# SingleZombie/AFLDM

Measured on AMD Instinct MI355X. Metric: denoise-steps/sec + ms/step, FFHQ-256 AF-UNet, batch 64 @1/2/4/8 GPU, higher is better.
Workload: dtype bf16; 1 GPU; FFHQ-256 AF-UNet single denoise step, batch 64 per GPU (BASELINE configs[1]); batch_per_gpu=64, global_batch=64, hip_graph=True, latents_finite=True

## Files before the change

afldm_amd/csrc/conv.hip:

```cpp
#include <stdlib.h>

#include "conv_common.hpp"

namespace afldm {

__device__ __forceinline__ int swz(int row) { return (4 - ((row >> 2) & 3)) & 3; }

template <typename T>
__device__ __forceinline__ void epilogue_store(const ConvP& p, int m, int n, f32x4 v) {
  const T* temb = (const T*)p.temb;
  const T* res = (const T*)p.residual;
  T* y = (T*)p.y;
  const int HW = p.H * p.W;
  const int b = m / HW;
  if (p.y2 && n >= p.split_n) {
    T* y2 = (T*)p.y2;
    const int pix = m - b * HW, c2 = p.Cout - p.split_n;
    for (int r = 0; r < 4 && n + r < p.Cout; ++r) {
      float sv = v[r] + (p.bias ? p.bias[n + r] : 0.f);
      y2[((size_t)b * c2 + (n + r - p.split_n)) * HW + pix] = from_f32<T>(sv);
    }
    return;
  }
  if (n + 3 < p.Cout && p.vec_ok) {
// ... 1845 lines not shown
    const int eo = 16 / (int)sizeof(T);
    const int hw = a->H * a->W;
    const bool cm = a->out_mode == 1 || a->y2;
    p.stage_ok = ((a->out_mode == 1 || a->y_ld % eo == 0) && (!a->residual || a->res_ld % eo == 0) &&
                  (!a->temb || a->temb_stride % eo == 0) && (!cm || hw % eo == 0) && (!a->y2 || a->split_n % eo == 0) &&
                  !(cm && a->residual)) ? 1 : 0;
    static const int s_nostage = getenv("AFLDM_CONV_NOSTAGE") ? atoi(getenv("AFLDM_CONV_NOSTAGE")) : 0;
    if (s_nostage) p.stage_ok = 0;
  }
  {
    static const int s_mfast = getenv("AFLDM_CONV_MFAST") ? atoi(getenv("AFLDM_CONV_MFAST")) : -1;
    p.m_fast = s_mfast >= 0 ? s_mfast : ((long long)a->Cout * a->KS * a->KS > (long long)p.M ? 1 : 0);
  }
  p.xcd_gn = 0;
  p.y_norm = nullptr; p.ngamma = nullptr; p.nbeta = nullptr; p.ncpg = 1; p.neps = 0.f;
  p.x_c8 = a->x_layout == 1 ? 1 : 0;
  p.y_c8 = a->y_layout == 1 ? 1 : 0;
  p.w_nt = 0;
  p.sc_x1 = a->sc_x1; p.sc_x2 = a->sc_x2; p.sc_w = a->sc_w;
  p.sc_C1 = a->sc_x1 ? a->sc_C1 : 0; p.sc_C2 = a->sc_x1 ? a->sc_C2 : 0;
}

template <typename T>
static bool shortcut_ok(const afldm_conv_args* a) {
  const int kstep = KCH_DEFAULT * epr<T>();
  const long long M = (long long)a->B * a->H * a->W, Csc = (long long)a->sc_C1 + a->sc_C2;
  if (!a->sc_x1 || !a->sc_w || a->sc_C1 <= 0 || a->sc_C2 < 0 || a->sc_C1 % kstep || a->sc_C2 % kstep || (a->sc_C2 > 0) != (a->sc_x2 != nullptr))
    return false;
  if (!aligned16(a->sc_x1) || !aligned16(a->sc_x2) || !aligned16(a->sc_w)) return false;
  if (a->KS != 3 || a->residual || a->defer_reduce || a->w_batch_stride || a->y_norm || a->y2 || a->out_mode != 0) return false;
  const long long cmax = a->sc_C1 > a->sc_C2 ? a->sc_C1 : a->sc_C2;
  if (M >= (1ll << 28) || M * cmax * (long long)sizeof(T) >= (1ll << 31) || (long long)a->Cout * Csc * (long long)sizeof(T) >= (1ll << 31)) return false;
  if (lin_wreg_bm(a) || skinny_stats_splits(a)) return false;
  const Exec ex = resolve_exec<T>(a);
  return ex.pl.kind == 0 && kVariants[ex.vid].ver == 6 && ex.splitk == 1 && !ex.fused && conv3h_shortcut_ok(ex.vid);
}

template <typename T>
static bool c8_ok(const afldm_conv_args* a) {
  if (sizeof(T) != 2 || a->C2 != 0 || a->x2 || a->y2 || a->out_mode != 0 || a->y_norm || a->y_ld != a->Cout || a->Cout % 8 || a->C1 % 64) return false;
  if (a->w_batch_stride || a->defer_reduce || a->KS != 3 || lin_wreg_bm(a) || skinny_stats_splits(a)) return false;
  const Exec ex = resolve_exec<T>(a);
  if (ex.pl.kind != 0 || kVariants[ex.vid].ver != 6 || ex.splitk != 1 || ex.fused) return false;
  if (a->stats_out) {
    int S = 0;
    if (stats_mode<T>(a, ex, &S) != ST_EPILOGUE) return false;
  }
  return a->H == a->W && a->W <= 32 && a->H * a->W >= kVariants[ex.vid].bm;
}

template <typename T>
static int conv_dispatch(const afldm_conv_args* a, hipStream_t st) {
  AFLDM_REQUIRE((a->x_layout == 0 && a->y_layout == 0) || c8_ok<T>(a), AFLDM_ESHAPE,
                "afldm_conv2d: x_layout / y_layout = 1 (8-channel blocks) is not available for this problem (afldm_conv2d_c8_ok)");
  AFLDM_REQUIRE(!a->sc_x1 || shortcut_ok<T>(a), AFLDM_ESHAPE,
                "afldm_conv2d: the folded shortcut (sc_x1 / sc_w) is not available for this problem (afldm_conv2d_shortcut_ok)");
  ConvP p;
  fill_convp<T>(a, p);
// ... 186 lines not shown
  const afldm_conv_args* a = &ac;
  const Exec e = a->dtype == AFLDM_F32 ? resolve_exec<float>(a) : resolve_exec<bf16>(a);
  if (skinny_stats_splits(a)) return -16;
  if (e.pl.kind != 0) return -1 - e.pl.kind;
  return e.vid | (e.splitk << 8) | (e.fused << 16);
}

extern "C" int afldm_conv2d_c8_ok(const afldm_conv_args* a) {
  if (!a || a->dtype != AFLDM_BF16 || conv_validate(a) || conv_batch_chunk(a) != a->B) return 0;
  return c8_ok<bf16>(a) ? 1 : 0;
}

extern "C" int afldm_conv2d_norm_ok(const afldm_conv_args* a) {
  if (!a || a->dtype != AFLDM_BF16 || conv_batch_chunk(a) != a->B || !a->stats_out) return 0;
  if (lin_wreg_bm(a) || skinny_stats_splits(a)) return 0;
  const Exec e = resolve_exec<bf16>(a);
  int S = 0;
  const int smode = stats_mode<bf16>(a, e, &S);
  return norm_fusable<bf16>(a, e, smode) ? 1 : 0;
}

extern "C" int afldm_conv2d_shortcut_ok(const afldm_conv_args* a) {
  if (!a || conv_validate(a) || conv_batch_chunk(a) != a->B) return 0;
  if (a->dtype == AFLDM_BF16) return shortcut_ok<bf16>(a) ? 1 : 0;
  if (a->dtype == AFLDM_F32) return shortcut_ok<float>(a) ? 1 : 0;
  return 0;
}

extern "C" int afldm_conv2d_stats_splits(const afldm_conv_args* a0) {
  if (!a0 || (a0->dtype != AFLDM_F32 && a0->dtype != AFLDM_BF16)) return 0;
  const afldm_conv_args ac = conv_chunk_args(a0, conv_batch_chunk(a0));
  const afldm_conv_args* a = &ac;
  int S = 0;
  if (a->dtype == AFLDM_F32) stats_mode<float>(a, resolve_exec<float>(a), &S);
  else stats_mode<bf16>(a, resolve_exec<bf16>(a), &S);
  return S;
}

extern "C" size_t afldm_conv2d_workspace(const afldm_conv_args* a0) {
  if (!a0 || (a0->dtype != AFLDM_F32 && a0->dtype != AFLDM_BF16)) return 0;
  const afldm_conv_args ac = conv_chunk_args(a0, conv_batch_chunk(a0));
  const afldm_conv_args* a = &ac;
  if (lin_wreg_bm(a) || skinny_stats_splits(a)) return 0;
  Plan pl = make_plan(a, a->dtype == AFLDM_F32 ? 16 : 32);
  if (pl.kind != 0 || pl.splitk <= 1) return 0;
  return (size_t)pl.splitk * a->B * a->H * a->W * a->Cout * sizeof(float);
}

// ... 30 lines not shown
```

afldm_amd/csrc/conv3h.hip:

```cpp
#include "conv3h_tile.hpp"

namespace afldm {

template <typename T, int BM, int W_, int BN, int WGM, int WGN, int NPROD, int STAGES, int MINW, int MF, int TPS, bool SUB = false>
__global__ void __launch_bounds__((WGM * WGN + NPROD) * 64, MINW) k_conv3h(ConvP p) {
  extern __shared__ __attribute__((aligned(16))) char smem[];
#define H3_BX blockIdx.x
#define H3_NBX gridDim.x
#define H3_BZ blockIdx.z
#define H3_PATCH_AUX 0
#define H3_PRODUCER_EXIT return;
#include "conv3h_body.inc"
#undef H3_PRODUCER_EXIT
#undef H3_BX
#undef H3_NBX
#undef H3_BZ
#undef H3_PATCH_AUX
}

template <int BM, int W_, int BN, int WGM, int WGN, bool SUB>
__global__ void __launch_bounds__((WGM * WGN + 4) * 64, (WGM * WGN + 4 + 3) / 4) k_conv3h_pers(ConvP p) {
  typedef bf16 T;
  typedef Mma<T> MM;
  typedef typename MM::Chunk Chunk;
// ... 374 lines not shown
  const int k = variant - kConv3hFirst;
  if (k < 0 || k >= kNumH3) return false;
  const H3Variant& v = kH3[k];
  if (v.bm == 0) return false;
  const int kstep = 128 / dtype_size;
  const int eo = 16 / dtype_size;
  const int HW = p.H * p.W;
  const int z = p.splitk > 0 ? p.splitk : 1;
  const bool tile_ok = HW % v.bm == 0 || (v.bm % HW == 0 && (z > 1 || dtype_size == 2));
  const bool plane_ok = v.sub ? (p.W > v.w && p.W % v.w == 0 && p.H % (v.bm / v.w) == 0 && z == 1) : (p.W == v.w && p.H == p.W && tile_ok);
  if ((k == 22 || k == 23) && !(dtype_size == 2 && z == 1 && HW % v.bm == 0 && p.C1 / kstep >= 2 && (!p.temb || p.temb_mod > 0))) return false;
  if (k >= 24 && dtype_size != 2) return false;
  return p.KS == 3 && p.C2 == 0 && plane_ok && p.M % v.bm == 0 && p.Cout % v.bn == 0 &&
         p.C1 % kstep == 0 && (p.C1 / kstep) % z == 0 && p.out_mode == 0 && !p.y2 && p.y_ld % eo == 0 &&
         (!p.residual || p.res_ld % eo == 0) && (!p.temb || (p.temb_stride % eo == 0 && p.temb_mod % eo == 0)) &&
         (long long)p.M * p.C1 * dtype_size < (1ll << 31) && (long long)p.Cout * 9 * p.C1 * dtype_size < (1ll << 31) &&
         p.Cout % 4 == 0 && aligned16(p.y) && aligned16(p.x1) && aligned16(p.w);
}

bool conv3h_shortcut_ok(int variant) {
  const int k = variant - kConv3hFirst;
  if (k < 0 || k >= kNumH3 || k == 22 || k == 23) return false;
  const H3Variant& v = kH3[k];
  return v.bm != 0 && v.tps == 1 && !v.sub && !(v.bm == 256 && v.w == 16);
}

template <typename T, int BM, int W_, int BN, int WGM, int WGN, int MF, int TPS, int STAGES = 3, bool SUB = false, int NPROD = 4, int MINW_ = 0>
static void launch_h3(const ConvP& p0, hipStream_t st) {
  constexpr int NWC = WGM * WGN;
  constexpr int MINW = MINW_ > 0 ? MINW_ : (NWC + NPROD + 3) / 4;
  constexpr int ROWS = BM / W_, SEG = ROWS < W_ ? ROWS : W_, NSEG = ROWS / SEG;
  constexpr int NPI = (NSEG * (SEG + 2) * (W_ + 2) + 7) / 8;
  constexpr int lds = 2 * NPI * 1024 + STAGES * TPS * BN * 128;
  static_assert(lds <= 160 * 1024, "LDS");
  ConvP p = p0;
  p.tiles_n = p.Cout / BN;
  if (p.splitk < 1) p.splitk = 1;
  const int tiles_m = p.M / BM, tiles = tiles_m * p.tiles_n;
  {
    static const int s_gn = getenv("AFLDM_CONV3H_GN") ? atoi(getenv("AFLDM_CONV3H_GN")) : -1;
    const double xb = (double)p.M * p.C1, wb = 9.0 * p.Cout * p.C1;
    int best = 0;
    double best_cost = xb + 8.0 * wb;
    for (int gn = 2; gn <= 8; gn *= 2) {
      if (tiles % 8 || p.tiles_n % gn || tiles_m % (8 / gn)) continue;
      const double c = xb * gn + wb * (8 / gn);
      if (c < 0.9 * best_cost) best = gn, best_cost = c;
// ... 81 lines not shown
```

afldm_amd/csrc/conv3h_body.inc:

```
  typedef Mma<T> MM;
  typedef typename MM::Chunk Chunk;
  constexpr int NWC = WGM * WGN;
  constexpr int EPC = MM::EPC, KSTEP = 8 * EPC, ESZ = (int)sizeof(T);
  constexpr int WMS = BM / WGM, WNS = BN / WGN, TM = WMS / MF, TN = WNS / MF;
  constexpr int ROWS = BM / W_, SEG = ROWS < W_ ? ROWS : W_, NSEG = ROWS / SEG;
  constexpr int PW = W_ + 2, PR = NSEG * (SEG + 2), NPQ = PR * PW, NPI = (NPQ + 7) / 8;
  constexpr int PATCH = NPI * 1024;
  constexpr int SPC = 9 / TPS;
  constexpr int WIT = BN / 8;
  constexpr int WI = TPS * WIT, WPW = WI / NPROD, PPW = (NPI + NPROD - 1) / NPROD;
  constexpr int W_TAP = BN * 128, W_STAGE = TPS * W_TAP;
  constexpr int LDS_TOTAL = 2 * PATCH + STAGES * W_STAGE;
  constexpr unsigned OOB = 0x80000000u;
  static_assert(MF == 16 || MF == 32, "MFMA flavour");
  static_assert(TPS == 1 || TPS == 3, "taps per step");
  static_assert(BM % W_ == 0 && ROWS % SEG == 0 && WI % NPROD == 0 && WMS % MF == 0 && WNS % MF == 0, "tile shape");
  static_assert((STAGES - 2) * WPW + PPW < 64, "vmcnt is a 6-bit counter");

  const int tid = threadIdx.x, lane = tid & 63;
  const int wave_all = __builtin_amdgcn_readfirstlane(tid >> 6);
  const bool is_producer = wave_all >= NWC;
  const int li = lane & (MF - 1), lg = lane / MF;

  int tile_m, tile_n;
  if (p.xcd_gn > 0) {
    const int xcd = H3_BX & 7, j = H3_BX >> 3;
    const int gn = p.xcd_gn, tn_per = p.tiles_n / gn, tm_per = (H3_NBX / p.tiles_n) / (8 / gn);
    const int xm = xcd / gn, xn = xcd - xm * gn;
    const int lm = j / tn_per, ln = j - lm * tn_per;
    tile_m = xm * tm_per + lm;
    tile_n = xn * tn_per + ln;
  } else {
    const int tile = xcd_remap(H3_BX, H3_NBX);
    tile_m = tile / p.tiles_n;
    tile_n = tile - tile_m * p.tiles_n;
  }
  static_assert(!SUB || (NSEG == 1 && TPS == 1), "sub-tiled planes: one segment per tile");
  const int n0 = tile_n * BN;
  const int Ct = p.C1, HW = SUB ? p.H * p.W : W_ * W_;
  const int ncb = Ct / KSTEP;
  const int ks = H3_BZ;
  const int cb_lo = (ncb * ks) / p.splitk, cb_hi = (ncb * (ks + 1)) / p.splitk;
  constexpr bool HAS_SC = TPS == 1 && !SUB && !(BM == 256 && W_ == 16);
  const int nsc = (HAS_SC && p.sc_x1) ? (p.sc_C1 + p.sc_C2) / KSTEP : 0;
  const int cb_end = cb_hi + nsc;
  const int Gm = (cb_hi - cb_lo) * SPC, G = Gm + nsc;
  int m0, b_tile, oh0, ow0 = 0, sp_tile;
  if constexpr (SUB) {
    const int tw = p.W / W_, tps = (p.H / ROWS) * tw;
    b_tile = tile_m / tps;
    sp_tile = tile_m - b_tile * tps;
    const int ty = sp_tile / tw;
    oh0 = ty * ROWS;
    ow0 = (sp_tile - ty * tw) * W_;
    m0 = b_tile * HW + oh0 * p.W + ow0;
  } else {
    m0 = tile_m * BM;
    b_tile = m0 / HW;
    oh0 = NSEG == 1 ? (m0 - b_tile * HW) / W_ : 0;
    sp_tile = (m0 - b_tile * HW) / BM;
  }
  auto gpix = [&](int tp) -> int {
    if constexpr (SUB) return m0 + (tp / W_) * p.W + (tp % W_);
    else return m0 + tp;
  };

  if (is_producer) {
// ... 22 lines not shown
        ok = q < NPQ && pc >= 1 && pc <= W_ && ih >= 0 && ih < W_;
        pixel = m0 + (sg * SEG + jj - 1) * W_ + (pc - 1);
      }
      if (p.x_c8) {
        const int bb = pixel / HW, pp = pixel - bb * HW;
        poff[i] = ok ? (((unsigned)(bb * (Ct / EPC) + c) * (unsigned)HW + (unsigned)pp) * (unsigned)EPC) * ESZ : OOB;
      } else {
        poff[i] = ok ? ((unsigned)pixel * (unsigned)Ct + (unsigned)(c * EPC)) * ESZ : OOB;
      }
    }
#pragma unroll
    for (int i = 0; i < WPW; ++i) {
      const int j = wave + NPROD * i;
      const int tis = j / WIT, r = 8 * (j - tis * WIT) + (lane >> 3);
      const int c = h_chunk_at<MF>(lane & 7, h_sw_rows<MF>(r));
      woff[i] = (((unsigned)(n0 + r) * 9u + (unsigned)tis) * (unsigned)Ct + (unsigned)(c * EPC)) * ESZ;
    }
    const int Csc = p.sc_C1 + p.sc_C2;
    __amdgpu_buffer_rsrc_t rws = __builtin_amdgcn_make_buffer_rsrc((void*)p.sc_w, 0, (int)((long long)p.Cout * Csc * ESZ), 0x00020000);
    int is_g = 0, is_st = 0, is_cb = cb_lo, is_slot = 0;
    auto issue_weights = [&]() {
      char* sbase = smem + 2 * PATCH + is_slot * W_STAGE;
      if (HAS_SC && is_g >= Gm && is_g < G) {
        const unsigned so = (unsigned)((is_g - Gm) * KSTEP * ESZ);
#pragma unroll
        for (int i = 0; i < WPW; ++i) {
          const int r = 8 * (wave + NPROD * i) + (lane >> 3);
          const unsigned wo = ((unsigned)(n0 + r) * (unsigned)Csc + (unsigned)(h_chunk_at<MF>(lane & 7, h_sw_rows<MF>(r)) * EPC)) * ESZ;
          lds_ptr_t dst = (lds_ptr_t)(sbase + (wave + NPROD * i) * 1024);
          if (p.w_nt) __builtin_amdgcn_raw_ptr_buffer_load_lds(rws, dst, 16, (int)wo, (int)so, 0, 2);
          else __builtin_amdgcn_raw_ptr_buffer_load_lds(rws, dst, 16, (int)wo, (int)so, 0, 0);
        }
      } else {
        const unsigned so = is_g < Gm ? (unsigned)((is_st * TPS * Ct + is_cb * KSTEP) * ESZ) : OOB;
#pragma unroll
        for (int i = 0; i < WPW; ++i) {
          lds_ptr_t dst = (lds_ptr_t)(sbase + (wave + NPROD * i) * 1024);
          if (p.w_nt) __builtin_amdgcn_raw_ptr_buffer_load_lds(rw, dst, 16, (int)woff[i], (int)so, 0, 2);
          else __builtin_amdgcn_raw_ptr_buffer_load_lds(rw, dst, 16, (int)woff[i], (int)so, 0, 0);
        }
      }
      ++is_g;
      if (++is_st == SPC) {
        is_st = 0;
        ++is_cb;
      }
      is_slot = is_slot + 1 == STAGES ? 0 : is_slot + 1;
    };
    auto issue_patch = [&](int cb) {
      char* sbase = smem + ((cb - cb_lo) & 1) * PATCH;
      if (HAS_SC && cb >= cb_hi) {
        const int c0 = (cb - cb_hi) * KSTEP;
        const bool in1 = c0 < p.sc_C1;
        const int Cs = in1 ? p.sc_C1 : p.sc_C2;
        __amdgpu_buffer_rsrc_t rs = __builtin_amdgcn_make_buffer_rsrc(const_cast<void*>(in1 ? p.sc_x1 : p.sc_x2), 0,
                                                                     (int)((long long)p.M * Cs * ESZ), 0x00020000);
        const unsigned so = (unsigned)((in1 ? c0 : c0 - p.sc_C1) * ESZ);
#pragma unroll
        for (int i = 0; i < PPW; ++i) {
          const int q = 8 * pj[i] + (lane >> 3);
          const int c = h_chunk_at<MF>(lane & 7, h_sw_patch<MF, W_>(q));
          const int pr = q / PW, pc = q - pr * PW;
          const int sg = pr / (SEG + 2), jj = pr - sg * (SEG + 2);
          const bool in = q < NPQ && pc >= 1 && pc <= W_ && jj >= 1 && jj <= SEG;
          const int pixel = m0 + (sg * SEG + jj - 1) * W_ + (pc - 1);
          const unsigned off = in ? ((unsigned)pixel * (unsigned)Cs + (unsigned)(c * EPC)) * ESZ : OOB;
          lds_ptr_t dst = (lds_ptr_t)(sbase + pj[i] * 1024);
          __builtin_amdgcn_raw_ptr_buffer_load_lds(rs, dst, 16, (int)off, (int)so, 0, 0);
        }
        return;
      }
      const unsigned so = p.x_c8 ? (unsigned)cb * (unsigned)(KSTEP * ESZ) * (unsigned)HW : (unsigned)(cb * KSTEP * ESZ);
#pragma unroll
      for (int i = 0; i < PPW; ++i) {
        lds_ptr_t dst = (lds_ptr_t)(sbase + pj[i] * 1024);
        __builtin_amdgcn_raw_ptr_buffer_load_lds(rx, dst, 16, (int)poff[i], (int)so, 0, H3_PATCH_AUX);
      }
    };
    issue_patch(cb_lo);
#pragma unroll
    for (int s = 0; s < STAGES - 1; ++s) issue_weights();
    int st = 0, cb = cb_lo, since = STAGES;
    bool fresh = false;
    for (int g = 0; g < G; ++g) {
      if (fresh) wait_vmcnt<(STAGES >= 3 ? WPW : 0)>();
      else if (since <= STAGES - 1) wait_vmcnt<(STAGES - 2) * WPW + PPW>();
      else wait_vmcnt<(STAGES - 2) * WPW>();
      __builtin_amdgcn_s_barrier();
      ++since;
      fresh = false;
      if (!(p.dbg & 1)) {
        if (HAS_SC && cb >= cb_hi) {
          if (cb + 1 < cb_end) {
            issue_patch(cb + 1);
            fresh = true;
            since = STAGES;
          }
          issue_weights();
        } else {
          issue_weights();
          if (st == 0 && cb + 1 < cb_end) {
            issue_patch(cb + 1);
            since = 1;
          }
        }
      }
      if ((HAS_SC && cb >= cb_hi) || ++st == SPC) {
        st = 0;
        ++cb;
      }
// ... 102 lines not shown
          }
#pragma unroll
          for (int kk = 0; kk < NKK; ++kk) {
            Chunk a[TN], b[TM];
#pragma unroll
            for (int t = 0; t < TN; ++t) a[t] = ld16<Chunk>(sW + ti * W_TAP + ((a_off0 + t * MF * 128) ^ (kk << 5)));
#pragma unroll
            for (int t = 0; t < TM; ++t) b[t] = ld16<Chunk>(sP + (bo[t] ^ (kk << 5)));
#pragma unroll
            for (int tn = 0; tn < TN; ++tn)
#pragma unroll
              for (int tm = 0; tm < TM; ++tm) {
                if constexpr (MF == 16) MM::mma(acc[tn][tm], a[tn], b[tm]);
                else Mma32<T>::mma(acc[tn][tm], a[tn], b[tm]);
              }
            __builtin_amdgcn_sched_barrier(0);
          }
        }
      }
      step_end();
    };
    auto k_step = [&](auto ST) {
      constexpr int sst = decltype(ST)::value;
      if (!(p.dbg & 2)) {
        const char* sP = smem + pbuf * PATCH;
        const char* sW = smem + 2 * PATCH + slot * W_STAGE;
        int boff[TPS][TM];
#pragma unroll
        for (int ti = 0; ti < TPS; ++ti) {
          const int tap = st * TPS + ti;
          const int tapoff = (tap / 3) * PW + (tap - (tap / 3) * 3);
#pragma unroll
          for (int t = 0; t < TM; ++t) {
            if constexpr (sst >= 0) boff[ti][t] = btab[sst * TPS + ti][t];
            else boff[ti][t] = frag_off(qb[t] + tapoff);
          }
        }
        constexpr int NPH = TPS * NKK, NG = NPH * TN, AD = 3;
        Chunk af[NG], bf[NPH][TM];
        auto lda = [&](int i) {
          const int ph = i / TN, ti = ph / NKK, kk = ph - ti * NKK;
#ifdef AFLDM_H3_NOLOAD
          return Chunk{};
#endif
          return ld16<Chunk>(sW + ti * W_TAP + ((a_off0 + (i - ph * TN) * MF * 128) ^ (kk << 5)));
        };
        auto ldb = [&](int ph, int t) {
          const int ti = ph / NKK, kk = ph - ti * NKK;
#ifdef AFLDM_H3_NOLOAD
          return Chunk{};
#endif
          return ld16<Chunk>(sP + (boff[ti][t] ^ (kk << 5)));
        };
#pragma unroll
        for (int t = 0; t < TM; ++t) bf[0][t] = ldb(0, t);
#pragma unroll
        for (int i = 0; i < AD; ++i) af[i] = lda(i);
        __builtin_amdgcn_sched_barrier(0);
#pragma unroll
        for (int i = 0; i < NG; ++i) {
          if (i + AD < NG) af[i + AD] = lda(i + AD);
// ... 23 lines not shown
        constexpr int c = decltype(C)::value;
        __builtin_amdgcn_s_barrier();
        if (c > 0) res_add(c - 1);
        res_issue(c);
        if constexpr (TPS == 3) k_step_plain(C);
        else k_step_plain(RT{});
      };
      static_assert(TPS == 1 || NRS == SPC, "peeled steps = one channel block");
      peeled(std::integral_constant<int, 0>{});
      peeled(std::integral_constant<int, 1>{});
      peeled(std::integral_constant<int, 2>{});
      if constexpr (NRS > 3) {
        peeled(std::integral_constant<int, 3>{});
        peeled(std::integral_constant<int, 4>{});
        peeled(std::integral_constant<int, 5>{});
        peeled(std::integral_constant<int, 6>{});
        peeled(std::integral_constant<int, 7>{});
      }
      static_assert(NRS == 3 || NRS == 8, "peeled steps");
      res_add(NRS - 1);
      g = NRS;
    }
    if constexpr (TPS == 3) {
      for (; g < G; g += 3) {
        __builtin_amdgcn_s_barrier();
        k_step(std::integral_constant<int, 0>{});
        __builtin_amdgcn_s_barrier();
        k_step(std::integral_constant<int, 1>{});
        __builtin_amdgcn_s_barrier();
        k_step(std::integral_constant<int, 2>{});
      }
    } else {
      for (; g < Gm; ++g) {
        __builtin_amdgcn_s_barrier();
        k_step(RT{});
      }
      for (; HAS_SC && g < G; ++g) {
        __builtin_amdgcn_s_barrier();
        st = 4;
        k_step(RT{});
        st = 0;
        pbuf ^= 1;
      }
    }
  }

  if (p.dbg & 8) return;
  if constexpr (ESZ == 2) {
    if (p.splitk == 1) {
      constexpr int NTC = NWC * 64, EO = 8, CPR = BN / EO, RPI = NTC / CPR, OROW = BN + 8;
      constexpr int SB_BYTES = ((NSEG * BN * 4 + 1023) / 1024) * 1024, HWT = BM / NSEG;
      static_assert(SB_BYTES + BM * OROW * 2 <= LDS_TOTAL && RPI * BN * 8 <= LDS_TOTAL, "staging tile");
      float* sB = reinterpret_cast<float*>(smem);
// ... 267 lines not shown
```

afldm_amd/csrc/conv_common.hpp:

```cpp
#pragma once
#include "common.hpp"

namespace afldm {

struct ConvP {
  const void* x1;
  const void* x2;
  const void* w;
  const float* bias;
  const void* temb;
  const void* residual;
  void* y;
  void* y2;
  float* ws;
  int split_n;
  int C1, C2, B, H, W, Cout, KS;
  int temb_stride, res_ld, y_ld, out_mode;
  int temb_mod;
  int M;
  int ksteps;
  int splitk;
  int tiles_n;
  int vec_ok;
  int tap_inner;
// ... 9 lines not shown
  void* y_norm;
  const float* ngamma;
  const float* nbeta;
  int ncpg;
  float neps;
  int x_c8, y_c8;
  int w_nt;
  const void* sc_x1;
  const void* sc_x2;
  const void* sc_w;
  int sc_C1, sc_C2;
};

typedef __attribute__((address_space(3))) void* lds_ptr_t;

template <int N>
__device__ __forceinline__ void wait_vmcnt() {
  asm volatile("s_waitcnt vmcnt(%0)" ::"n"(N) : "memory");
}

constexpr int kConv3hFirst = 41;
bool conv3h_supported(int variant, int dtype_size, const ConvP& p);
bool conv3h_shortcut_ok(int variant);
int conv3h_tile(int variant, int* bm, int* bn);
void conv3h_launch(int variant, int dtype_size, const ConvP& p, hipStream_t st);
bool conv3h_plan(const afldm_conv_args* a, ConvP* p, int* variant);

}
```

afldm_amd/models/blocks.py:

```python
import math

import os

import torch
import torch.nn as nn

from .. import aql, ops

_SC_ORDER = int(os.environ.get("AFLDM_SHORTCUT_ORDER", "0"))
_C8_EDGES = int(os.environ.get("AFLDM_C8_EDGES", "5"))
_SC_FOLD = os.environ.get("AFLDM_NO_SHORTCUT_FOLD", "0") != "1"


def _pair(x):
    return x if isinstance(x, tuple) else (x, None)


class PackedMixin:

    def _packed(self, key, build):
        cache = self.__dict__.setdefault("_afldm_cache", {})
        if key not in cache:
            cache[key] = build()
        return cache[key]

    def _invalidate(self):
        self.__dict__.pop("_afldm_cache", None)


def invalidate_packed(module: nn.Module):
    for m in module.modules():
        m.__dict__.pop("_afldm_cache", None)


# ... 338 lines not shown
        cin = x1.shape[-1] + (0 if x2 is None else x2.shape[-1])
        key = (B, N, cin, x1.device, int(temb_stride))
        cache = self.__dict__.setdefault("_afldm_c8", {})
        if key not in cache:
            w1, b1 = packed_conv(self.conv1, x1.dtype)
            w2, b2 = packed_conv(self.conv2, x1.dtype)
            a_in = torch.empty((B, N, N, cin), dtype=x1.dtype, device=x1.device)
            h_in = torch.empty((B, N, N, self.out_channels), dtype=x1.dtype, device=x1.device)
            cache[key] = (ops.conv2d_c8_ok(a_in, w1, b1, temb=temb_proj, temb_stride=temb_stride),
                          ops.conv2d_c8_ok(h_in, w2, b2, residual=h_in))
        return cache[key]

    def _sc_bias(self):
        cache = self.__dict__.setdefault("_afldm_cache", {})
        if "sc_bias" not in cache:
            b = torch.zeros(self.out_channels, dtype=torch.float64, device=self.conv2.weight.device)
            for conv in (self.conv2, self.conv_shortcut):
                if conv.bias is not None:
                    b += conv.bias.detach().double()
            cache["sc_bias"] = b.float().contiguous()
        return cache["sc_bias"]

    def _sc_fold_plan(self, input_tensor, c8):
        if (not _SC_FOLD or self.conv_shortcut is None or tuple(self.conv_shortcut.kernel_size) != (1, 1)
                or tuple(self.conv2.kernel_size) != (3, 3)):
            return False
        x1, x2 = _pair(input_tensor)
        if x1.ndim != 4 or x1.shape[1] != x1.shape[2]:
            return False
        B, N = x1.shape[0], x1.shape[1]
        key = (B, N, x1.shape[-1], None if x2 is None else x2.shape[-1], x1.dtype, x1.device, bool(c8))
        cache = self.__dict__.setdefault("_afldm_sc_fold", {})
        if key not in cache:
            w2, _ = packed_conv(self.conv2, x1.dtype)
            wsc, _ = packed_conv(self.conv_shortcut, x1.dtype)
            h_in = torch.empty((B, N, N, self.out_channels), dtype=x1.dtype, device=x1.device)
            if c8:
                h_in.c8 = True
            cache[key] = ops.conv2d_shortcut_ok(h_in, w2, self._sc_bias(), (x1, x2, wsc))
        return cache[key]

    def _conv2_sc_folded(self, h, input_tensor, next_gn):
        x1, x2 = _pair(input_tensor)
        w2, _ = packed_conv(self.conv2, h.dtype)
        wsc, _ = packed_conv(self.conv_shortcut, h.dtype)
        kw = {}
        if next_gn is not None:
            gamma, beta = packed_norm(next_gn)
            kw["norm_out"] = (gamma, beta, next_gn.num_groups, next_gn.eps)
        out = ops.conv2d(h, w2, self._sc_bias(), want_stats=True, shortcut=(x1, x2, wsc), **kw)
        hn = getattr(out, "norm_applied", None)
        if hn is not None:
            out.gn_applied = (hn, next_gn)
        return out

    def _norm_act(self, norm, x, out_c8=False, out_const=False):
        from ..af_modules.af_blocks import WarpedNonlinearity
        x1, x2 = _pair(x)
        gamma, beta = packed_norm(norm)
        stats = ops.gn_stats(x1, norm.num_groups, x2=x2)
        if isinstance(self.nonlinearity, WarpedNonlinearity):
            if self.nonlinearity.fused_silu:
                return ops.af_act(x1, x2, stats, gamma, beta, norm.num_groups, norm.eps, out_c8=out_c8, out_const=out_const)
            return self.nonlinearity(ops.gn_apply(x1, stats, gamma, beta, norm.num_groups, norm.eps, act=0, x2=x2))
        return ops.gn_apply(x1, stats, gamma, beta, norm.num_groups, norm.eps, act=1, x2=x2)

    def _norm_act_conv(self, norm, x, conv, force=False, **kw):
        from ..af_modules.af_blocks import WarpedNonlinearity
        x1, x2 = _pair(x)
        if (isinstance(self.nonlinearity, WarpedNonlinearity) and self.nonlinearity.fused_silu and x1.ndim == 4
# ... 13 lines not shown
            return None
        B, N, _, Cin = h.shape
        conv, norm = self.conv1, self.norm2
        Cout = conv.out_channels
        if tuple(conv.kernel_size) != (3, 3) or Cout % norm.num_groups or Cin % 8 or Cout % 8:
            return None
        if N == 2 and not os.environ.get("AFLDM_NO_DENSE2X2"):
            w2, _ = packed_conv_dense2x2(conv, h.dtype, Cin, 0)
            got = ops.conv2d_slabs(h.reshape(B, 4 * Cin), w2)
        else:
            w, _ = packed_conv(conv, h.dtype)
            got = ops.conv2d_slabs(h, w)
        if got is None:
            return None
        slabs, nslab = got
        gamma, beta = packed_norm(norm)
        cache = conv.__dict__.setdefault("_afldm_cache", {})
        if "bias_f32" not in cache:
            cache["bias_f32"] = None if conv.bias is None else conv.bias.detach().to(torch.float32).contiguous()
        bias = cache["bias_f32"]
        return ops.af_act_slabs(slabs, nslab, bias, temb_proj, temb_stride, gamma, beta, norm.num_groups, norm.eps,
                                B, N, Cout, h.dtype)

    def _conv2_to_next_norm_fused(self, h, res, next_gn):
        if (os.environ.get("AFLDM_NO_FUSED_ACT") or isinstance(h, tuple) or h.ndim != 4 or h.shape[1] != h.shape[2]
                or h.shape[1] not in (2, 4)):
            return None
        B, N, _, Cin = h.shape
        conv = self.conv2
        Cout = conv.out_channels
        if (tuple(conv.kernel_size) != (3, 3) or Cout % next_gn.num_groups or Cin % 8 or Cout % 8
                or next_gn.num_channels != Cout or res.shape[-1] != Cout or not res.is_contiguous()):
            return None
        if N == 2 and not os.environ.get("AFLDM_NO_DENSE2X2"):
            w2, _ = packed_conv_dense2x2(conv, h.dtype, Cin, 0)
            got = ops.conv2d_slabs(h.reshape(B, 4 * Cin), w2)
        else:
            w, _ = packed_conv(conv, h.dtype)
            got = ops.conv2d_slabs(h, w)
        if got is None:
            return None
        slabs, nslab = got
        gamma, beta = packed_norm(next_gn)
        cache = conv.__dict__.setdefault("_afldm_cache", {})
        if "bias_f32" not in cache:
            cache["bias_f32"] = None if conv.bias is None else conv.bias.detach().to(torch.float32).contiguous()
        hn, y = ops.af_act_slabs(slabs, nslab, cache["bias_f32"], None, 0, gamma, beta, next_gn.num_groups, next_gn.eps,
                                 B, N, Cout, h.dtype, residual=res, want_raw=True, act=False)
        y.gn_applied = (hn, next_gn)
        return y

    def _const2_ok(self, input_tensor):
        from ..af_modules.af_blocks import WarpedNonlinearity
        x1, x2 = _pair(input_tensor)
        return (_CONST2 and not os.environ.get("AFLDM_NO_DENSE2X2") and x1.ndim == 4 and x1.shape[1] == 2 and x1.shape[2] == 2
                and isinstance(self.nonlinearity, WarpedNonlinearity) and self.nonlinearity.fused_silu
                and tuple(self.conv1.kernel_size) == (3, 3) and tuple(self.conv2.kernel_size) == (3, 3)
                and x1.shape[-1] % 8 == 0 and (x2 is None or x2.shape[-1] % 8 == 0) and self.out_channels % 8 == 0
                and self.out_channels % self.norm2.num_groups == 0
                and (x1.shape[-1] + (0 if x2 is None else x2.shape[-1])) % (128 // x1.element_size()) == 0
                and self.out_channels % (128 // x1.element_size()) == 0)

    def _forward_const2(self, input_tensor, temb_proj, temb_stride, next_gn):
        x1, x2 = _pair(input_tensor)
        B, dt, Cout = x1.shape[0], x1.dtype, self.out_channels
        a = self._norm_act(self.norm1, input_tensor, out_const=True)
        g2, be2 = packed_norm(self.norm2)
        h = None
        got = None
        if ops.conv2x2_const_norm_act_ok(a.shape[-1], Cout, self.norm2.num_groups, dt, batch=B) and not os.environ.get("AFLDM_NO_FUSED_ACT"):
# ... 297 lines not shown
```

afldm_amd/ops.py:

```python
import ctypes
import os

import torch

from . import _exp, _lib
from ._lib import AfActArgs, ConvArgs, DTYPE_CODE, SepArgs, check, stream_ptr

_FILTER_CACHE = {}
_PROFILE = None


class _RecordingLib:

    def __init__(self, raw):
        self._raw = raw
        self._wrapped = {}

    def __getattr__(self, name):
        w = self._wrapped.get(name)
        if w is None:
            f = getattr(self._raw, name)

            def w(*a, _f=f):
                if _PROFILE is not None:
# ... 652 lines not shown
    key = (tuple(x1.shape), tuple(w.shape), temb is not None, int(temb_stride), residual is not None, bool(want_stats), str(x1.device))
    if key not in _C8_OK:
        a = conv_args(x1, w, bias, None, temb, temb_stride, residual, None)
        a.y = ptr(x1)
        if want_stats and w.shape[0] % 4 == 0:
            a.stats_out = ptr(x1)
        a.x_layout = 0
        _C8_OK[key] = (not lib.afldm_conv2d_workspace(ctypes.byref(a))) and bool(lib.afldm_conv2d_c8_ok(ctypes.byref(a)))
    return _C8_OK[key]


_C8_OK = {}


def _set_shortcut(a, shortcut):
    sx1, sx2, sw = shortcut
    _dev(sx1, "shortcut x1")
    assert not is_c8(sx1) and not is_c8(sx2), "the folded shortcut reads NHWC tensors"
    a.sc_x1, a.sc_x2, a.sc_w = ptr(sx1), ptr(sx2), ptr(sw)
    a.sc_C1, a.sc_C2 = sx1.shape[-1], 0 if sx2 is None else sx2.shape[-1]
    a.keep = a.keep + (sx1, sx2, sw)


def conv2d_shortcut_ok(x1, w, bias, shortcut, temb=None, temb_stride=0, want_stats=True):
    sx1, sx2, sw = shortcut
    if x1.ndim != 4 or sx1.ndim != 4 or w.shape[1] != 3 or sw.shape[1] != 1:
        return False
    key = (tuple(x1.shape), is_c8(x1), x1.dtype, tuple(w.shape), tuple(sx1.shape), None if sx2 is None else tuple(sx2.shape),
           temb is not None, int(temb_stride), bool(want_stats), str(x1.device))
    if key not in _SC_OK:
        a = conv_args(x1, w, bias, None, temb, temb_stride, None, None)
        a.y = ptr(sx1)
        if want_stats and w.shape[0] % 4 == 0:
            a.stats_out = ptr(sx1)
        _set_shortcut(a, shortcut)
        _SC_OK[key] = (not lib.afldm_conv2d_workspace(ctypes.byref(a))) and bool(lib.afldm_conv2d_shortcut_ok(ctypes.byref(a)))
    return _SC_OK[key]


_SC_OK = {}


def conv2d(x1, w, bias=None, x2=None, temb=None, temb_stride=0, residual=None, out=None, out_mode=0,
           workspace=None, want_stats=False, temb_mod=0, w_batch_stride=0, norm_out=None, out_c8=False, shortcut=None):
    Cout = w.shape[0]
    if out is None:
        if out_mode == 0:
            out = torch.empty(tuple(x1.shape[:-1]) + (Cout,), dtype=x1.dtype, device=x1.device)
        else:
            B = x1.shape[0]
            out = torch.empty((B, Cout, x1.numel() // (B * x1.shape[-1])), dtype=x1.dtype, device=x1.device)
    a = conv_args(x1, w, bias, x2, temb, temb_stride, residual, out, out_mode, workspace, temb_mod=temb_mod)
    if out_c8:
        a.y_layout = 1
        out.c8 = True
    a.w_batch_stride = int(w_batch_stride)
    if shortcut is not None:
        _set_shortcut(a, shortcut)
    if out_mode == 1 and x1.ndim == 3:
# ... 113 lines not shown
        _end(tok, name, fl, by, replay=replay)
    if pre is not None:
        out.act_input = act_out
    return out, post_out


def af_act_conv2d(x1, x2, stats, gamma, beta, G, eps, w, bias=None, temb=None, temb_stride=0, residual=None,
                  want_stats=False):
    got = act_conv_act(x1, x2, (stats, gamma, beta, G, eps), w, bias, temb, temb_stride, residual, want_stats)
    return None if got is None else got[0]


def actconv_error(device=None):
    worst = 0
    bufs = [b for (dev, _), b in _SYNC.items() if device is None or dev == str(device)] + [r() for r in _SCOPED_SYNC if r() is not None]
    for buf in bufs:
        v = int(buf[8193].item())
        if v:
            worst = max(worst, v)
            buf[8193] = 0
    return worst


def conv2d_slabs(x1, w, x2=None):
    Cout = w.shape[0]
    out = torch.empty(tuple(x1.shape[:-1]) + (Cout,), dtype=x1.dtype, device=x1.device)
    a = conv_args(x1, w, None, x2, out=out)
    need = lib.afldm_conv2d_workspace(ctypes.byref(a))
    if not need:
        return None
    workspace = torch.empty(need // 4, dtype=torch.float32, device=x1.device)
    a.workspace, a.workspace_bytes = ptr(workspace), need
    code = lib.afldm_conv2d_variant(ctypes.byref(a))
    nslab = (code >> 8) & 255 if code >= 0 else 1
    if code < 0 or nslab <= 1 or (code >> 16) & 1 or need < nslab * a.B * a.H * a.W * Cout * 4:
        return None
    a.defer_reduce = 1
    a.keep = a.keep + (workspace,)
    tok = _begin()
    check(lib.afldm_conv2d(ctypes.byref(a), stream_ptr()), "conv2d(slabs)")
    if tok is not None:
        M, Ct = a.B * a.H * a.W, a.C1 + a.C2
        es = x1.element_size()
        kind = "conv3x3" if a.KS == 3 else ("conv1x1" if a.H * a.W > 1 and x1.ndim == 4 else "linear")
        keep = (a, workspace, out)
        _end(tok, kind, 2.0 * M * a.Cout * a.KS * a.KS * Ct, (M * Ct + a.Cout * a.KS * a.KS * Ct + M * a.Cout) * es,
             replay=lambda keep=keep: conv2d_launch(keep[0]))
    return workspace[:nslab * a.B * a.H * a.W * Cout].view(nslab, a.B * a.H * a.W, Cout), nslab


def af_act_slabs(slabs, nslab, bias, temb, temb_stride, gamma, beta, G, eps, B, N, C, dtype, residual=None, want_raw=False,
                 act=True):
    const = act == 2
    assert not const or N == 2
    out = torch.empty((B, C) if const else (B, N, N, C), dtype=dtype, device=slabs.device)
    raw = torch.empty((B, N, N, C), dtype=dtype, device=slabs.device) if want_raw else None
    U, D = filter_matrices(N, slabs.device)
    tok = _begin()
    check(lib.afldm_af_act_slabs(ptr(slabs), int(nslab), ptr(bias), ptr(temb), int(temb_stride), ptr(residual), ptr(raw),
                                 ptr(gamma), ptr(beta), int(G), float(eps), 2 if const else (1 if act else 0), ptr(U), ptr(D),
                                 ptr(out), B, C, N, _code(out), stream_ptr()), "af_act_slabs")
    if const:
        out.const2 = True
    _end(tok, f"af_act_N{N}" if act else "gn_apply", 24.0 * N ** 3 * B * C if act else 0.0,
         B * N * N * C * (4 * nslab + out.element_size() * (2 if want_raw else 1)))
    return (out, raw) if want_raw else out


_DENSE2_MIN_B = int(os.environ.get("AFLDM_DENSE2_MIN_B", "64"))
# ... 497 lines not shown
```

Measured before the change: 14070 denoise-steps/s.

## Fold 1x1 shortcut conv into three-taps-per-step split-K conv3x3 slab path

Extends the shortcut-fold fusion, where the 1x1 residual shortcut conv is computed as extra K-steps inside the 3x3 conv2 kernel, to the TPS=3 kernel variants. Those shortcut K-steps are now split across split-K slices and fed into the deferred-reduce slab path with the fused GroupNorm apply. The kernel gets a single-tap k_step variant and per-stage vmcnt waits that account for the smaller shortcut weight loads. The point is to remove a separate 1x1 conv launch and residual-add pass for blocks that use split-K or 3-tap tiles, at the cost of extra kernel complexity and new wait-count logic that could be fragile.

Measured after the change: 14260 denoise-steps/s, median of 6. 1.01x the previous value.

```diff
diff --git a/afldm_amd/csrc/conv.hip b/afldm_amd/csrc/conv.hip
--- a/afldm_amd/csrc/conv.hip
+++ b/afldm_amd/csrc/conv.hip
@@ -1891,18 +1891,20 @@
 }
 
 template <typename T>
-static bool shortcut_ok(const afldm_conv_args* a) {
+static int shortcut_ok(const afldm_conv_args* a) {
   const int kstep = KCH_DEFAULT * epr<T>();
   const long long M = (long long)a->B * a->H * a->W, Csc = (long long)a->sc_C1 + a->sc_C2;
   if (!a->sc_x1 || !a->sc_w || a->sc_C1 <= 0 || a->sc_C2 < 0 || a->sc_C1 % kstep || a->sc_C2 % kstep || (a->sc_C2 > 0) != (a->sc_x2 != nullptr))
-    return false;
-  if (!aligned16(a->sc_x1) || !aligned16(a->sc_x2) || !aligned16(a->sc_w)) return false;
-  if (a->KS != 3 || a->residual || a->defer_reduce || a->w_batch_stride || a->y_norm || a->y2 || a->out_mode != 0) return false;
+    return 0;
+  if (!aligned16(a->sc_x1) || !aligned16(a->sc_x2) || !aligned16(a->sc_w)) return 0;
+  if (a->KS != 3 || a->residual || a->w_batch_stride || a->y2 || a->out_mode != 0) return 0;
   const long long cmax = a->sc_C1 > a->sc_C2 ? a->sc_C1 : a->sc_C2;
-  if (M >= (1ll << 28) || M * cmax * (long long)sizeof(T) >= (1ll << 31) || (long long)a->Cout * Csc * (long long)sizeof(T) >= (1ll << 31)) return false;
-  if (lin_wreg_bm(a) || skinny_stats_splits(a)) return false;
+  if (M >= (1ll << 28) || M * cmax * (long long)sizeof(T) >= (1ll << 31) || (long long)a->Cout * Csc * (long long)sizeof(T) >= (1ll << 31)) return 0;
+  if (lin_wreg_bm(a) || skinny_stats_splits(a)) return 0;
   const Exec ex = resolve_exec<T>(a);
-  return ex.pl.kind == 0 && kVariants[ex.vid].ver == 6 && ex.splitk == 1 && !ex.fused && conv3h_shortcut_ok(ex.vid);
+  if (ex.pl.kind != 0 || kVariants[ex.vid].ver != 6 || ex.fused || !conv3h_shortcut_ok(ex.vid)) return 0;
+  if (conv3h_taps_per_step(ex.vid) == 3) return (a->defer_reduce && ex.splitk == 1) ? 0 : 2;
+  return (ex.splitk == 1 && !a->defer_reduce && !a->y_norm) ? 1 : 0;
 }
 
 template <typename T>
@@ -2135,8 +2137,8 @@
 
 extern "C" int afldm_conv2d_shortcut_ok(const afldm_conv_args* a) {
   if (!a || conv_validate(a) || conv_batch_chunk(a) != a->B) return 0;
-  if (a->dtype == AFLDM_BF16) return shortcut_ok<bf16>(a) ? 1 : 0;
-  if (a->dtype == AFLDM_F32) return shortcut_ok<float>(a) ? 1 : 0;
+  if (a->dtype == AFLDM_BF16) return shortcut_ok<bf16>(a);
+  if (a->dtype == AFLDM_F32) return shortcut_ok<float>(a);
   return 0;
 }
 
diff --git a/afldm_amd/csrc/conv3h.hip b/afldm_amd/csrc/conv3h.hip
--- a/afldm_amd/csrc/conv3h.hip
+++ b/afldm_amd/csrc/conv3h.hip
@@ -420,7 +420,12 @@
   const int k = variant - kConv3hFirst;
   if (k < 0 || k >= kNumH3 || k == 22 || k == 23) return false;
   const H3Variant& v = kH3[k];
-  return v.bm != 0 && v.tps == 1 && !v.sub && !(v.bm == 256 && v.w == 16);
+  return v.bm != 0 && !v.sub && !(v.bm == 256 && v.w == 16) && !(v.tps == 3 && v.bn == 48);
+}
+
+int conv3h_taps_per_step(int variant) {
+  const int k = variant - kConv3hFirst;
+  return (k < 0 || k >= kNumH3) ? 0 : kH3[k].tps;
 }
 
 template <typename T, int BM, int W_, int BN, int WGM, int WGN, int MF, int TPS, int STAGES = 3, bool SUB = false, int NPROD = 4, int MINW_ = 0>
diff --git a/afldm_amd/csrc/conv3h_body.inc b/afldm_amd/csrc/conv3h_body.inc
--- a/afldm_amd/csrc/conv3h_body.inc
+++ b/afldm_amd/csrc/conv3h_body.inc
@@ -9,6 +9,7 @@
   constexpr int SPC = 9 / TPS;
   constexpr int WIT = BN / 8;
   constexpr int WI = TPS * WIT, WPW = WI / NPROD, PPW = (NPI + NPROD - 1) / NPROD;
+  constexpr int WPS = WPW / TPS;
   constexpr int W_TAP = BN * 128, W_STAGE = TPS * W_TAP;
   constexpr int LDS_TOTAL = 2 * PATCH + STAGES * W_STAGE;
   constexpr unsigned OOB = 0x80000000u;
@@ -16,6 +17,7 @@
   static_assert(TPS == 1 || TPS == 3, "taps per step");
   static_assert(BM % W_ == 0 && ROWS % SEG == 0 && WI % NPROD == 0 && WMS % MF == 0 && WNS % MF == 0, "tile shape");
   static_assert((STAGES - 2) * WPW + PPW < 64, "vmcnt is a 6-bit counter");
+  static_assert(TPS == 1 || (STAGES == 3 && WIT % NPROD == 0), "three taps per step: a wave's first WPS instructions are the stage's first tap slot");
 
   const int tid = threadIdx.x, lane = tid & 63;
   const int wave_all = __builtin_amdgcn_readfirstlane(tid >> 6);
@@ -41,8 +43,10 @@
   const int ncb = Ct / KSTEP;
   const int ks = H3_BZ;
   const int cb_lo = (ncb * ks) / p.splitk, cb_hi = (ncb * (ks + 1)) / p.splitk;
-  constexpr bool HAS_SC = TPS == 1 && !SUB && !(BM == 256 && W_ == 16);
-  const int nsc = (HAS_SC && p.sc_x1) ? (p.sc_C1 + p.sc_C2) / KSTEP : 0;
+  constexpr bool HAS_SC = !SUB && !(BM == 256 && W_ == 16) && !(TPS == 3 && BN == 48);
+  const int nsc_all = (HAS_SC && p.sc_x1) ? (p.sc_C1 + p.sc_C2) / KSTEP : 0;
+  const int sc_lo = TPS == 3 ? (nsc_all * ks) / p.splitk : 0;
+  const int nsc = TPS == 3 ? (nsc_all * (ks + 1)) / p.splitk - sc_lo : nsc_all;
   const int cb_end = cb_hi + nsc;
   const int Gm = (cb_hi - cb_lo) * SPC, G = Gm + nsc;
   int m0, b_tile, oh0, ow0 = 0, sp_tile;
@@ -111,9 +115,9 @@
     auto issue_weights = [&]() {
       char* sbase = smem + 2 * PATCH + is_slot * W_STAGE;
       if (HAS_SC && is_g >= Gm && is_g < G) {
-        const unsigned so = (unsigned)((is_g - Gm) * KSTEP * ESZ);
-#pragma unroll
-        for (int i = 0; i < WPW; ++i) {
+        const unsigned so = (unsigned)((sc_lo + is_g - Gm) * KSTEP * ESZ);
+#pragma unroll
+        for (int i = 0; i < WPS; ++i) {
           const int r = 8 * (wave + NPROD * i) + (lane >> 3);
           const unsigned wo = ((unsigned)(n0 + r) * (unsigned)Csc + (unsigned)(h_chunk_at<MF>(lane & 7, h_sw_rows<MF>(r)) * EPC)) * ESZ;
           lds_ptr_t dst = (lds_ptr_t)(sbase + (wave + NPROD * i) * 1024);
@@ -139,7 +143,7 @@
     auto issue_patch = [&](int cb) {
       char* sbase = smem + ((cb - cb_lo) & 1) * PATCH;
       if (HAS_SC && cb >= cb_hi) {
-        const int c0 = (cb - cb_hi) * KSTEP;
+        const int c0 = (sc_lo + cb - cb_hi) * KSTEP;
         const bool in1 = c0 < p.sc_C1;
         const int Cs = in1 ? p.sc_C1 : p.sc_C2;
         __amdgpu_buffer_rsrc_t rs = __builtin_amdgcn_make_buffer_rsrc(const_cast<void*>(in1 ? p.sc_x1 : p.sc_x2), 0,
@@ -172,9 +176,21 @@
     int st = 0, cb = cb_lo, since = STAGES;
     bool fresh = false;
     for (int g = 0; g < G; ++g) {
-      if (fresh) wait_vmcnt<(STAGES >= 3 ? WPW : 0)>();
-      else if (since <= STAGES - 1) wait_vmcnt<(STAGES - 2) * WPW + PPW>();
-      else wait_vmcnt<(STAGES - 2) * WPW>();
+      if constexpr (TPS == 1) {
+        if (fresh) wait_vmcnt<(STAGES >= 3 ? WPW : 0)>();
+        else if (since <= STAGES - 1) wait_vmcnt<(STAGES - 2) * WPW + PPW>();
+        else wait_vmcnt<(STAGES - 2) * WPW>();
+      } else {
+        const bool sc_next = HAS_SC && g + 1 >= Gm && g + 1 < G;
+        const bool patch_behind = !fresh && since <= STAGES - 1;
+        if (sc_next) {
+          if (patch_behind) wait_vmcnt<WPS + PPW>();
+          else wait_vmcnt<WPS>();
+        } else {
+          if (patch_behind) wait_vmcnt<WPW + PPW>();
+          else wait_vmcnt<WPW>();
+        }
+      }
       __builtin_amdgcn_s_barrier();
       ++since;
       fresh = false;
@@ -323,21 +339,23 @@
     };
     auto k_step = [&](auto ST) {
       constexpr int sst = decltype(ST)::value;
+      constexpr int NT = sst == -2 ? 1 : TPS;
       if (!(p.dbg & 2)) {
         const char* sP = smem + pbuf * PATCH;
         const char* sW = smem + 2 * PATCH + slot * W_STAGE;
-        int boff[TPS][TM];
-#pragma unroll
-        for (int ti = 0; ti < TPS; ++ti) {
+        int boff[NT][TM];
+#pragma unroll
+        for (int ti = 0; ti < NT; ++ti) {
           const int tap = st * TPS + ti;
           const int tapoff = (tap / 3) * PW + (tap - (tap / 3) * 3);
 #pragma unroll
           for (int t = 0; t < TM; ++t) {
             if constexpr (sst >= 0) boff[ti][t] = btab[sst * TPS + ti][t];
+            else if constexpr (sst == -2) boff[ti][t] = btab[TPS == 3 ? 4 : 0][t];
             else boff[ti][t] = frag_off(qb[t] + tapoff);
           }
         }
-        constexpr int NPH = TPS * NKK, NG = NPH * TN, AD = 3;
+        constexpr int NPH = NT * NKK, NG = NPH * TN, AD = 3;
         Chunk af[NG], bf[NPH][TM];
         auto lda = [&](int i) {
           const int ph = i / TN, ti = ph / NKK, kk = ph - ti * NKK;
@@ -407,13 +425,21 @@
       g = NRS;
     }
     if constexpr (TPS == 3) {
-      for (; g < G; g += 3) {
+      for (; g < Gm; g += 3) {
         __builtin_amdgcn_s_barrier();
         k_step(std::integral_constant<int, 0>{});
         __builtin_amdgcn_s_barrier();
         k_step(std::integral_constant<int, 1>{});
         __builtin_amdgcn_s_barrier();
         k_step(std::integral_constant<int, 2>{});
+      }
+      if constexpr (HAS_SC) {
+        for (; g < G; ++g) {
+          __builtin_amdgcn_s_barrier();
+          k_step(std::integral_constant<int, -2>{});
+          st = 0;
+          pbuf ^= 1;
+        }
       }
     } else {
       for (; g < Gm; ++g) {
diff --git a/afldm_amd/csrc/conv_common.hpp b/afldm_amd/csrc/conv_common.hpp
--- a/afldm_amd/csrc/conv_common.hpp
+++ b/afldm_amd/csrc/conv_common.hpp
@@ -55,6 +55,7 @@
 constexpr int kConv3hFirst = 41;
 bool conv3h_supported(int variant, int dtype_size, const ConvP& p);
 bool conv3h_shortcut_ok(int variant);
+int conv3h_taps_per_step(int variant);
 int conv3h_tile(int variant, int* bm, int* bn);
 void conv3h_launch(int variant, int dtype_size, const ConvP& p, hipStream_t st);
 bool conv3h_plan(const afldm_conv_args* a, ConvP* p, int* variant);
diff --git a/afldm_amd/models/blocks.py b/afldm_amd/models/blocks.py
--- a/afldm_amd/models/blocks.py
+++ b/afldm_amd/models/blocks.py
@@ -10,6 +10,7 @@
 _SC_ORDER = int(os.environ.get("AFLDM_SHORTCUT_ORDER", "0"))
 _C8_EDGES = int(os.environ.get("AFLDM_C8_EDGES", "5"))
 _SC_FOLD = os.environ.get("AFLDM_NO_SHORTCUT_FOLD", "0") != "1"
+_SC_FOLD3 = os.environ.get("AFLDM_NO_SHORTCUT_FOLD3", "0") != "1"
 
 
 def _pair(x):
@@ -394,7 +395,7 @@
         return cache["sc_bias"]
 
     def _sc_fold_plan(self, input_tensor, c8):
-        if (not _SC_FOLD or self.conv_shortcut is None or tuple(self.conv_shortcut.kernel_size) != (1, 1)
+        if ((not _SC_FOLD and not _SC_FOLD3) or self.conv_shortcut is None or tuple(self.conv_shortcut.kernel_size) != (1, 1)
                 or tuple(self.conv2.kernel_size) != (3, 3)):
             return False
         x1, x2 = _pair(input_tensor)
@@ -402,15 +403,26 @@
             return False
         B, N = x1.shape[0], x1.shape[1]
         key = (B, N, x1.shape[-1], None if x2 is None else x2.shape[-1], x1.dtype, x1.device, bool(c8))
-        cache = self.__dict__.setdefault("_afldm_sc_fold", {})
-        if key not in cache:
+
+        def kind():
             w2, _ = packed_conv(self.conv2, x1.dtype)
             wsc, _ = packed_conv(self.conv_shortcut, x1.dtype)
             h_in = torch.empty((B, N, N, self.out_channels), dtype=x1.dtype, device=x1.device)
             if c8:
                 h_in.c8 = True
-            cache[key] = ops.conv2d_shortcut_ok(h_in, w2, self._sc_bias(), (x1, x2, wsc))
-        return cache[key]
+            return ops.conv2d_shortcut_ok(h_in, w2, self._sc_bias(), (x1, x2, wsc))
+        if _SC_FOLD:
+            cache = self.__dict__.setdefault("_afldm_sc_fold", {})
+            if key not in cache:
+                cache[key] = kind() == 1
+            if cache[key]:
+                return True
+        if _SC_FOLD3:
+            cache = self.__dict__.setdefault("_afldm_sc_fold3", {})
+            if key not in cache:
+                cache[key] = kind() == 2
+            return cache[key]
+        return False
 
     def _conv2_sc_folded(self, h, input_tensor, next_gn):
         x1, x2 = _pair(input_tensor)
@@ -418,6 +430,9 @@
         wsc, _ = packed_conv(self.conv_shortcut, h.dtype)
         kw = {}
         if next_gn is not None:
+            out = self._conv2_to_next_norm_fused(h, None, next_gn, shortcut=(x1, x2, wsc))
+            if out is not None:
+                return out
             gamma, beta = packed_norm(next_gn)
             kw["norm_out"] = (gamma, beta, next_gn.num_groups, next_gn.eps)
         out = ops.conv2d(h, w2, self._sc_bias(), want_stats=True, shortcut=(x1, x2, wsc), **kw)
@@ -477,17 +492,22 @@
         return ops.af_act_slabs(slabs, nslab, bias, temb_proj, temb_stride, gamma, beta, norm.num_groups, norm.eps,
                                 B, N, Cout, h.dtype)
 
-    def _conv2_to_next_norm_fused(self, h, res, next_gn):
+    def _conv2_to_next_norm_fused(self, h, res, next_gn, shortcut=None):
         if (os.environ.get("AFLDM_NO_FUSED_ACT") or isinstance(h, tuple) or h.ndim != 4 or h.shape[1] != h.shape[2]
                 or h.shape[1] not in (2, 4)):
             return None
         B, N, _, Cin = h.shape
         conv = self.conv2
         Cout = conv.out_channels
-        if (tuple(conv.kernel_size) != (3, 3) or Cout % next_gn.num_groups or Cin % 8 or Cout % 8
-                or next_gn.num_channels != Cout or res.shape[-1] != Cout or not res.is_contiguous()):
+        if (tuple(conv.kernel_size) != (3, 3) or Cout % next_gn.num_groups or Cin % 8 or Cout % 8 or next_gn.num_channels != Cout
+                or (shortcut is None and (res.shape[-1] != Cout or not res.is_contiguous()))):
             return None
-        if N == 2 and not os.environ.get("AFLDM_NO_DENSE2X2"):
+        if shortcut is not None:
+            w, _ = packed_conv(conv, h.dtype)
+            if N == 2 or ops.conv2d_shortcut_ok(h, w, None, shortcut, slabs=True) != 2:
+                return None
+            got = ops.conv2d_slabs(h, w, shortcut=shortcut)
+        elif N == 2 and not os.environ.get("AFLDM_NO_DENSE2X2"):
             w2, _ = packed_conv_dense2x2(conv, h.dtype, Cin, 0)
             got = ops.conv2d_slabs(h.reshape(B, 4 * Cin), w2)
         else:
@@ -500,7 +520,8 @@
         cache = conv.__dict__.setdefault("_afldm_cache", {})
         if "bias_f32" not in cache:
             cache["bias_f32"] = None if conv.bias is None else conv.bias.detach().to(torch.float32).contiguous()
-        hn, y = ops.af_act_slabs(slabs, nslab, cache["bias_f32"], None, 0, gamma, beta, next_gn.num_groups, next_gn.eps,
+        hn, y = ops.af_act_slabs(slabs, nslab, self._sc_bias() if shortcut is not None else cache["bias_f32"], None, 0, gamma, beta,
+                                 next_gn.num_groups, next_gn.eps,
                                  B, N, Cout, h.dtype, residual=res, want_raw=True, act=False)
         y.gn_applied = (hn, next_gn)
         return y
diff --git a/afldm_amd/ops.py b/afldm_amd/ops.py
--- a/afldm_amd/ops.py
+++ b/afldm_amd/ops.py
@@ -698,19 +698,23 @@
     a.keep = a.keep + (sx1, sx2, sw)
 
 
-def conv2d_shortcut_ok(x1, w, bias, shortcut, temb=None, temb_stride=0, want_stats=True):
+def conv2d_shortcut_ok(x1, w, bias, shortcut, temb=None, temb_stride=0, want_stats=True, slabs=False):
     sx1, sx2, sw = shortcut
     if x1.ndim != 4 or sx1.ndim != 4 or w.shape[1] != 3 or sw.shape[1] != 1:
-        return False
+        return 0
     key = (tuple(x1.shape), is_c8(x1), x1.dtype, tuple(w.shape), tuple(sx1.shape), None if sx2 is None else tuple(sx2.shape),
-           temb is not None, int(temb_stride), bool(want_stats), str(x1.device))
+           temb is not None, int(temb_stride), bool(want_stats), bool(slabs), str(x1.device))
     if key not in _SC_OK:
-        a = conv_args(x1, w, bias, None, temb, temb_stride, None, None)
+        a = conv_args(x1, w, None if slabs else bias, None, temb, temb_stride, None, None)
         a.y = ptr(sx1)
-        if want_stats and w.shape[0] % 4 == 0:
+        if want_stats and not slabs and w.shape[0] % 4 == 0:
             a.stats_out = ptr(sx1)
         _set_shortcut(a, shortcut)
-        _SC_OK[key] = (not lib.afldm_conv2d_workspace(ctypes.byref(a))) and bool(lib.afldm_conv2d_shortcut_ok(ctypes.byref(a)))
+        need = lib.afldm_conv2d_workspace(ctypes.byref(a))
+        if need:
+            a.workspace, a.workspace_bytes = ptr(sx1), need
+        a.defer_reduce = 1 if slabs else 0
+        _SC_OK[key] = int(lib.afldm_conv2d_shortcut_ok(ctypes.byref(a))) if (need or not slabs) else 0
     return _SC_OK[key]
 
 
@@ -870,10 +874,12 @@
     return worst
 
 
-def conv2d_slabs(x1, w, x2=None):
+def conv2d_slabs(x1, w, x2=None, shortcut=None):
     Cout = w.shape[0]
     out = torch.empty(tuple(x1.shape[:-1]) + (Cout,), dtype=x1.dtype, device=x1.device)
     a = conv_args(x1, w, None, x2, out=out)
+    if shortcut is not None:
+        _set_shortcut(a, shortcut)
     need = lib.afldm_conv2d_workspace(ctypes.byref(a))
     if not need:
         return None
@@ -892,7 +898,8 @@
         es = x1.element_size()
         kind = "conv3x3" if a.KS == 3 else ("conv1x1" if a.H * a.W > 1 and x1.ndim == 4 else "linear")
         keep = (a, workspace, out)
-        _end(tok, kind, 2.0 * M * a.Cout * a.KS * a.KS * Ct, (M * Ct + a.Cout * a.KS * a.KS * Ct + M * a.Cout) * es,
+        Csc = a.sc_C1 + a.sc_C2 if shortcut is not None else 0
+        _end(tok, kind, 2.0 * M * a.Cout * (a.KS * a.KS * Ct + Csc), (M * (Ct + Csc) + a.Cout * (a.KS * a.KS * Ct + Csc) + M * a.Cout) * es,
              replay=lambda keep=keep: conv2d_launch(keep[0]))
     return workspace[:nslab * a.B * a.H * a.W * Cout].view(nslab, a.B * a.H * a.W, Cout), nslab
 
```
